# atoptima/DynamicSparseArrays.jl

Measured on AMD Instinct MI355X. Metric: spmv_gbps_10M_nnz_pcsr, higher is better.
Workload: dtype f64; 1 GPU; C3: PCSR 1000000x1000000 Float64, 10000000 nnz per GPU, dense-x SpMV y=A*x (gather over the rowmajor twin); capacity_slots=16777216, physical_slot_bytes=12, collective=none

## Files before the change

### dynamicsparsearrays.jl_amd/csrc/dsa_dev.h

```cpp
#pragma once
#include <hip/hip_runtime.h>
#include <stdint.h>
#include <functional>
#include <mutex>

namespace dsa {

constexpr int WAVE = 64;
constexpr int64_t SEM_KEY = 0;
constexpr int MAX_LEVELS = 48;
constexpr int TABLE_PEND_MAX = 1024;
constexpr int64_t VIEW_SMALL_SLOTS = 65536;

struct KeyArr {
    void* p;
    int32_t wide;
    int32_t pad_;
#if defined(__HIPCC__)
    struct Ref {
        void* p; int32_t wide; int64_t i;
        __device__ __forceinline__ operator int64_t() const {
            return wide ? static_cast<const int64_t*>(p)[i] : (int64_t) static_cast<const int32_t*>(p)[i];
        }
        __device__ __forceinline__ void operator=(int64_t k) const {
// ... 196 lines not shown
hipError_t launch_permute(KeyArr src_keys, const double* src_vals, const uint64_t* src_occ, int64_t src_cap,
                          KeyArr dst_keys, double* dst_vals, const uint64_t* dst_occ, int64_t dst_cap, int64_t n0,
                          const Op* ops, int64_t i0, int64_t* sems, RebalanceWork* wsrc, RebalanceWork* wdst, hipStream_t stream);
hipError_t launch_compact_range(KeyArr keys, const double* vals, const uint64_t* occ, int64_t from, int64_t to,
                                KeyArr out_keys, double* out_vals, int64_t out_cap, RebalanceWork* work, int64_t* count,
                                hipStream_t stream);
hipError_t launch_spx_accum(const SlotView& V, const int64_t* xi, const double* xv, int64_t nx, double* acc, uint64_t* bm, int64_t ny,
                            hipStream_t stream);
hipError_t launch_spx_repair(const SlotView& V, const double* xd, const double* xf, int64_t nx, const double* pattern, double* y, int64_t ny,
                             hipStream_t stream);
hipError_t launch_spx_pattern_bits(const double* pattern, int64_t ny, uint64_t* bm, hipStream_t stream);
hipError_t launch_spx_finish(uint64_t* bm, int64_t ny, uint32_t* tile_cnt, uint32_t* tile_off, unsigned int* ticket, double* src, int clear_src,
                             int64_t* out_i, double* out_v, int64_t cap, int64_t* d_count, long long* host, int64_t pin_cells,
                             unsigned long long seq, hipStream_t stream);
hipError_t launch_scatter_x(const int64_t* xi, const double* xv, int64_t nx, double* xd, double* xf, int64_t nxd, hipStream_t stream);
hipError_t launch_packed_equal(KeyArr ka, const double* va, KeyArr kb, const double* vb, int64_t n, int32_t* differ, hipStream_t stream);
hipError_t launch_merge_axpby(KeyArr ka, const double* va, int64_t na, double alpha, KeyArr kb, const double* vb, int64_t nb,
                              double beta, int64_t* mk, double* mv, uint64_t* keep, hipStream_t stream);
hipError_t launch_widen_keys(const void* src32, void* dst64, int64_t n, hipStream_t stream);
hipError_t launch_store_ctl(Ctl* d_ctl, const Ctl& ctl, hipStream_t stream);
hipError_t launch_init_fresh(uint64_t* occ0, uint64_t* occ1, int64_t occ_words, unsigned long long* status, int64_t status_words,
                             Ctl* d_ctl, const Ctl& ctl, hipStream_t stream);
hipError_t launch_clear_occ(uint64_t* occ, int64_t from, int64_t to, hipStream_t stream);

hipError_t pool_alloc(void** out, size_t bytes);
void pool_free(void* p);
void pool_trim(size_t keep_bytes);
size_t pool_idle_bytes();
hipError_t pinned_alloc(void** out, size_t bytes);
void pinned_free(void* p);
hipError_t stream_get(hipStream_t* out);
void stream_put(hipStream_t s, int device);

struct BuildScratch {
    int64_t n = 0;
    void* base = nullptr; hipStream_t stream = nullptr;
    void* base_val = nullptr;
    void* d_ctl = nullptr; void* h_ctl = nullptr;
    uint32_t* ghist = nullptr; uint32_t* hist = nullptr; uint32_t* cnt_c = nullptr; uint32_t* cnt_p = nullptr;
    uint64_t* comp[2] = {nullptr, nullptr}; double* val[2] = {nullptr, nullptr};
    void* queue = nullptr;
    int64_t kmin = 0, pmin = 0; int kbits = 0, pbits = 0, sorted = 0; const double* vsorted = nullptr;
    int ibits = 0;
    bool wide_path = false;
    uint32_t *idx2 = nullptr, *fpart = nullptr, *fcell = nullptr, *spart = nullptr, *scell = nullptr;
    int64_t *p2 = nullptr, *k2 = nullptr;
};
struct KeyRange { int64_t lo = 0, hi = -1; bool known() const { return hi >= lo; } };
hipError_t device_key_scan(const int64_t* d_a, const int64_t* d_b, int64_t n, KeyRange* ra, KeyRange* rb, bool* a_zero, bool* b_zero,
                           hipStream_t stream);
hipError_t launch_key_scan_acc(const int64_t* d_a, const int64_t* d_b, int64_t n, long long* d_acc, hipStream_t stream);
hipError_t build_prepare(const int64_t* d_part, const int64_t* d_key, const double* d_val, int64_t nnz, KeyRange part_range, KeyRange key_range,
                         BuildScratch& s, int64_t counts[2], hipStream_t stream, const std::function<void()>* while_sorting = nullptr);
hipError_t build_emit(const double* d_val, int32_t combine, BuildScratch& s, KeyArr out_keys, double* out_vals,
                      int64_t* part_keys, int mode, int64_t nparts_explicit, hipStream_t stream, bool wait_and_free = true,
                      uint64_t* der_comp = nullptr, double* der_val = nullptr);
hipError_t build_derived_alloc(BuildScratch& s, int64_t n, int kbits, int pbits, int64_t kmin, int64_t pmin, hipStream_t stream);
hipError_t build_derived_sort(BuildScratch& s, int64_t counts[2], hipStream_t stream, const std::function<void()>* while_sorting = nullptr);
void build_abort(BuildScratch& s);
hipError_t launch_build_small_vec(int64_t* io, int n, int cap, int32_t combine, KeyArr out_k, double* out_v, unsigned long long seq, hipStream_t stream);

hipError_t launch_sequencer(KeyArr keys, double* vals, uint64_t* occ, int64_t* sems, int64_t* col_keys,
                            uint8_t* col_live, Ctl* ctl, const Op* ops, int64_t n_ops, int64_t n_avail, bool run_ok, const uint64_t* breaks,
                            Ctl* host_ctl, unsigned long long* host_seq, unsigned int seq,
                            hipStream_t stream);
hipError_t launch_op_breaks(const Op* ops, int64_t n, int mode, uint64_t* breaks, hipStream_t stream);
hipError_t launch_make_ops(const int64_t* a, const int64_t* b, const double* v, int32_t kind, int64_t n, Op* ops, hipStream_t stream);
size_t append_run_memo_bytes();
hipError_t launch_append_run(uint64_t* occ, Ctl* ctl, int64_t i0, int64_t R, const uint64_t* flags, const int64_t* d_T,
                             uint64_t* saved_memo, const int64_t* m3_out, hipStream_t stream);
hipError_t launch_append_model3(uint64_t* occ, Ctl* ctl, int64_t R, const uint64_t* flags, const int64_t* d_T, int64_t* out, hipStream_t stream);
hipError_t launch_append_model5(uint64_t* occ, Ctl* ctl, int64_t R, const uint64_t* flags, const int64_t* d_T, int64_t* out, hipStream_t stream);
hipError_t launch_run_expand(const Op* ops, int64_t i0, int64_t R, const Ctl* ctl, int64_t* col_keys, uint8_t* col_live, Op* cells,
                             uint64_t* flags, int64_t* out, hipStream_t stream);

struct TableMerge {
    int64_t* sems2; int64_t* keys2;
    int64_t* pkey; int64_t* pdst; int64_t* psem;
    int64_t* hdr;
};
hipError_t launch_table_merge(int64_t* sems, int64_t* col_keys, uint8_t* col_live, double* vals, Ctl* ctl, TableMerge tm, int64_t table_cap,
                              hipStream_t stream);

struct Plan {
    int64_t lo, hi;
    int64_t pos, aux;
    int64_t ws, we;
    int32_t count;
    int32_t action;
};
struct RoundState {
    int64_t cursor;
    int64_t limit;
    int32_t G;
    int32_t d;
    int32_t stop;
    int32_t min_prefix, G_next, pad;
    uint32_t ticket;
    int32_t ema;
    int64_t rounds, par_ops;
    int64_t why[8];
    int32_t tight;
    int32_t seq;
    int64_t cursor_n;
    int64_t pend0;
    int32_t np, np_n;
    int32_t cur, cur_n;
    int32_t run_ahead;
    int32_t drain;
    int64_t deferred;
};
struct PendOp { int64_t op; int32_t zlo, zhi; };
struct BurstPublish { RoundState* host_rs; Ctl* host_ctl; unsigned long long* host_seq; };
constexpr int FP_MODE_SETS = 0x100, FP_MODE_SHADOW = 0x200;
constexpr size_t FP_BYTES_PER_OP = 160;
constexpr int ROUND_GMAX = 1024;
struct BurstGraph {
    hipGraphExec_t exec = nullptr; hipGraph_t graph = nullptr; hipStream_t stream = nullptr;
    const void* key[12] = {};
    bool disabled = false;
    hipStream_t failed_on = nullptr;
};
struct DevBufs { void* keys; double* vals; uint64_t* occ; int64_t* sems; int64_t* col_keys; uint8_t* col_live; int32_t wide, pad; PendOp* pend;  };
hipError_t launch_burst(const DevBufs* bufs, Ctl* ctl, const Op* ops, RoundState* rs, Plan* plans, int rounds, BurstGraph* cache,
                        BurstPublish pub, hipStream_t stream);
void burst_graph_destroy(BurstGraph* cache);
hipError_t launch_local_rounds(const DevBufs* bufs, Ctl* ctl, const Op* ops, RoundState* rs, int max_rounds, BurstPublish pub, hipStream_t stream);

hipError_t launch_get_batch(int mode, const SlotView& V, const int64_t* qa, const int64_t* qb, int64_t n, double* out, int32_t* err_out,
                            hipStream_t stream);
hipError_t launch_get_small(int mode, const SlotView& V, int64_t* io, int n, unsigned long long seq, hipStream_t stream);
enum DbgRawOp : int32_t { DBG_FIND = 0, DBG_FIND_FAST = 1, DBG_INSERT = 2, DBG_INSERT_FAST = 3, DBG_DELETE = 4, DBG_DELETE_FAST = 5,
                          DBG_PURGE = 6, DBG_REBALANCE = 7 };
hipError_t launch_dbg_raw_block(KeyArr keys, double* vals, uint64_t* occ, int64_t* sems, int64_t len, int op, int64_t key, double val,
                                int64_t from, int64_t to, int64_t m, int64_t* out, hipStream_t stream);
hipError_t launch_dbg_raw_wave(KeyArr keys, double* vals, uint64_t* occ, int64_t* sems, int64_t len, int op, int64_t key, double val,
                               int64_t from, int64_t to, int64_t m, int64_t* out, hipStream_t stream);
hipError_t launch_check(const SlotView& V, int64_t occ_words, unsigned long long* report, hipStream_t stream);
hipError_t launch_view_small(const SlotView& V, int64_t col, KeyArr out_k, double* out_v, int64_t out_cap, int64_t* meta, int64_t* host,
                             int64_t host_cells, unsigned long long seq, int64_t range_from, int64_t range_to, hipStream_t stream);
hipError_t launch_partition_range(const SlotView& V, int64_t col, int64_t* out, hipStream_t stream);

hipError_t launch_spmv_gather(const SlotView& V, const double* x, int64_t nx, double* y, int64_t ny, int pattern, int mode, hipStream_t stream);
constexpr int SPMV_ZFILL = 1;
constexpr int SPMV_PLAIN_STREAM = 2;
constexpr int64_t SPMV_SPAN_SLOTS = 512;
constexpr int SPMV_META_BLOCKS = 1024;
constexpr int SPMV_META_WORDS = 3 * SPMV_META_BLOCKS + 1;
hipError_t launch_spmv_meta(const SlotView& V, unsigned long long* scratch, unsigned long long* out6_pinned, unsigned long long seq, hipStream_t stream);
constexpr int PLAN_GROUP_SHIFT = 12;
constexpr int64_t PLAN_GROUP_SLOTS = int64_t(1) << PLAN_GROUP_SHIFT;
constexpr int PLAN_ROWS = 1024;
constexpr int PLAN_MAX_SLICES = 63;
constexpr int64_t PLAN_MAX_GROUPS = 4096;
constexpr int PLAN_DESC = 5;
struct PlanDev {
    uint32_t* cell; double* val;
    uint32_t* off;
    uint32_t* cnt;
    uint32_t* gbase;
    uint32_t* pfirst;
    uint32_t* nsem;
    uint32_t* yrow;
    int64_t groups, width, cap_cells;
    int32_t slices, pad_;
};
hipError_t launch_spmv_plan_build(const SlotView& V, int64_t nx, int64_t ny, const PlanDev& pl, unsigned long long* out3_pinned,
                                  unsigned long long seq, hipStream_t stream);
hipError_t launch_spmv_plan(const PlanDev& pl, int64_t table_len, const double* x, double* y, int64_t ny, hipStream_t stream);
hipError_t launch_spmv_scatter(const SlotView& V, const double* x, int64_t nx, double* y, int64_t ny, hipStream_t stream);

}
```

### dynamicsparsearrays.jl_amd/csrc/dsa_host.hip

```cpp
#include "host.h"

#include <dlfcn.h>

#include <algorithm>
#include <chrono>
#include <cstdlib>
#include <cstring>
#include <string>
#include <vector>

using namespace dsa;
using namespace dsa::host;

namespace {
thread_local std::string g_err;
}

namespace dsa {
namespace host {
Roctx::Roctx() {
    const char* e = getenv("DSA_ROCTX");
    if (!(e && e[0] == '1')) return;
    for (const char* n : {"librocprofiler-sdk-roctx.so.1", "librocprofiler-sdk-roctx.so", "libroctx64.so.4", "libroctx64.so"}) {
        void* lib = dlopen(n, RTLD_NOW | RTLD_GLOBAL);
        if (!lib) continue;
        push = reinterpret_cast<int (*)(const char*)>(dlsym(lib, "roctxRangePushA"));
        pop = reinterpret_cast<int (*)()>(dlsym(lib, "roctxRangePop"));
        if (push && pop) return;
        push = nullptr; pop = nullptr;
    }
}
const Roctx& roctx() { static const Roctx r; return r; }
}
}

namespace dsa {
static const char* const k_dev_switches[] = {
    "DSA_BUILD_WIDE",
    "DSA_COUNT_MODEL",
    "DSA_DBG_RUN", "DSA_DBG_SPLIT", "DSA_DBG_TIME",
    "DSA_DBG_MOVE2",
    "DSA_FAIL_BUILD",
    "DSA_FP_MODE",
    "DSA_KEYS_WIDE",
    "DSA_LOCAL_ROUNDS",
    "DSA_MODEL3",
    "DSA_MODEL5",
    "DSA_PARBATCH",
    "DSA_POS_WIDE",
    "DSA_RUN_AHEAD",
    "DSA_SPMV_PLAN",
    "DSA_SPMV_SHARE", "DSA_SPMV_STREAM",
    "DSA_SPX_XDRIVEN",
    "DSA_TIGHT",
};
const char* dev_env(const char* name) {
#ifndef NDEBUG
    bool known = false;
    for (const char* s : k_dev_switches) known = known || std::strcmp(s, name) == 0;
    if (!known) { fprintf(stderr, "dev_env: %s is not in the table of development switches\n", name); abort(); }
#endif
#ifndef DSA_DEV
    const char* on = getenv("DSA_DEV");
    if (!(on && on[0] == '1')) return nullptr;
#endif
    return getenv(name);
}

hipError_t wait_pinned_seq(const volatile void* word, uint64_t want, hipStream_t s, uint64_t mask) {
    const volatile unsigned long long* w = static_cast<const volatile unsigned long long*>(word);
    auto published = [&] { return (__atomic_load_n(w, __ATOMIC_ACQUIRE) & mask) == want; };
    auto next_query = std::chrono::steady_clock::now() + std::chrono::milliseconds(2);
    while (!published()) {
        if (std::chrono::steady_clock::now() < next_query) continue;
        const hipError_t q = hipStreamQuery(s);
        if (q == hipErrorNotReady) { next_query = std::chrono::steady_clock::now() + std::chrono::milliseconds(2); continue; }
        if (q != hipSuccess) return q;
        if (!published()) return hipErrorUnknown;
    }
    return hipSuccess;
}
void set_last_error(const char* msg) { g_err = msg ? msg : ""; }
}

namespace {

constexpr size_t PENDING_FLUSH = 1u << 16;

Pma& orient(dsa_mat* h, int32_t o) {
    if (!h->has_major) fail(DSA_EMODE, "matrix is in fill mode");
    if (o != DSA_COLMAJOR && o != DSA_ROWMAJOR) fail(DSA_EARG, "orientation must be 0 or 1");
    return o == DSA_COLMAJOR ? h->col : h->row;
}

void vec_apply(dsa_vec_t* h, const int64_t* keys, const double* vals, int64_t n) {
    int32_t err = 0;
    static const bool par = [] { const char* e = dev_env("DSA_PARBATCH"); return !(e && e[0] == '0'); }();
    int64_t done;
    if (par && n >= 128) done = run_ops_parallel(h->P, OpBatch(OP_VEC_SET, keys, nullptr, vals, n), &err);
    else {
        std::vector<Op> ops((size_t)n);
        for (int64_t i = 0; i < n; ++i) ops[(size_t)i] = make_op(OP_VEC_SET, keys[i], 0, vals[i]);
        done = run_ops(h->P, ops, &err);
    }
    const int64_t upto = err ? std::min(done + 1, n) : done;
    for (int64_t i = 0; i < upto; ++i) if (vals[i] != 0.0) h->n = std::max(h->n, keys[i]);
    if (err) fail(err, err_text(err));
}
void vec_flush(dsa_vec_t* h) {
    bind_device(h->P);
    if (h->pk.empty()) return;
    std::vector<int64_t> k; std::vector<double> v;
    k.swap(h->pk); v.swap(h->pv);
    vec_apply(h, k.data(), v.data(), (int64_t)k.size());
}

int64_t vec_pack_alt(dsa_vec_t* h) {
    Pma& P = h->P;
    int64_t cnt = 0;
    const int alt = 1 - P.cur;
    {
        const int64_t c = pack_small(P, P.K(), P.V(), P.O(), 1, P.capacity(), P.KA(alt), P.vals[alt], P.cap_alloc);
        if (c >= 0) return c;
    }
    LAUNCH("compact", launch_compact_range(P.K(), P.V(), P.O(), 1, P.capacity(), P.KA(alt), P.vals[alt], P.cap_alloc, &P.work, &cnt, P.stream));
    return cnt;
}
void wait_for_pack(dsa_vec_t* producer, dsa_vec_t* consumer) {
    if (producer->P.stream == consumer->P.stream) return;
    HIPCHK(hipStreamSynchronize(producer->P.stream));
}

dsa_vec* vec_from_packed_dev(Pma& S, int64_t n, int64_t len) {
    auto* v = new dsa_vec();
    hipStream_t own = nullptr;
    try {
        pma_init_common(v->P, false, false);
        Pma& P = v->P;
        own = P.stream; P.stream = S.stream;
        P.wide = S.wide;
        const int64_t capacity = capacity_for(n);
        set_geometry_for_new(P, capacity, n);
        ensure_capacity_alloc(P, 2 * capacity, false);
        ++P.layout_epoch; ++P.stat_grid_rebalances;
        P.h_ctl->stat_rebalances = 0; P.h_ctl->stat_window_slots = 0;
        if (capacity != P.h_ctl->segment_capacity) { P.h_ctl->stat_rebalances = 1; P.h_ctl->stat_window_slots = capacity; }
        LAUNCH("init", launch_init_fresh(P.occ[0], P.occ[1], P.occ_words, P.work.status, P.work.status_cap, P.d_ctl, *P.h_ctl, P.stream));
        const int salt = 1 - S.cur;
        LAUNCH("rebalance", launch_rebalance(S.KA(salt), S.vals[salt], S.occ[salt], 1, n, true, P.K(), P.V(), P.O(), 1, capacity, n,
                                             nullptr, &P.work, P.stream));
        P.occ_dirty[P.cur] = (capacity + 63) / 64;
        if (S.ev_handoff == nullptr) HIPCHK(hipEventCreateWithFlags(&S.ev_handoff, hipEventDisableTiming));
        HIPCHK(hipEventRecord(S.ev_handoff, S.stream));
        HIPCHK(hipStreamWaitEvent(own, S.ev_handoff, 0));
        P.stream = own;
    } catch (...) {
        if (own) { (void)hipStreamSynchronize(v->P.stream); v->P.stream = own; }
        pma_destroy(v->P); delete v; throw;
    }
    v->n = len;
    return v;
}

}

namespace dsa {
namespace host {

void ensure_xy(dsa_mat* h, int64_t nx, int64_t ny) {
    if (nx > h->x_cap) { if (h->d_x) hipFree(h->d_x); h->x_cap = std::max<int64_t>(nx, 1024); HIPCHK(hipMalloc(&h->d_x, (size_t)h->x_cap * sizeof(double))); }
    if (ny > h->y_cap) { if (h->d_y) hipFree(h->d_y); h->y_cap = std::max<int64_t>(ny, 1024); HIPCHK(hipMalloc(&h->d_y, (size_t)h->y_cap * sizeof(double))); }
}

void spmv_dev(dsa_mat* h, int32_t transpose, int32_t algo, const double* d_x, int64_t nx, double* d_y, int64_t ny, hipStream_t s,
              int pattern) {
    if (!h->has_major) fail(DSA_EMODE, "matrix is in fill mode");
    hipError_t e;
    if (algo == 0) {
        Pma& P = transpose ? h->col : h->row;
        int mode = 0;
        constexpr int64_t MAX_FILL = 4096;
        const Pma::SpmvMeta& M = spmv_meta(P);
        if (M.ordered && M.max_extent <= SPMV_SPAN_SLOTS && M.max_gap <= MAX_FILL && M.first_key >= 1 && M.first_key <= MAX_FILL &&
            ny - M.last_key <= MAX_FILL)
            { mode |= SPMV_ZFILL; ++P.stat_spmv_nomemset; }
        if (nx * (int64_t)sizeof(double) <= (3 << 20)) mode |= SPMV_PLAIN_STREAM;
        const bool plan = spmv_plan_on() && pattern == 0 && (mode & SPMV_ZFILL) && !(mode & SPMV_PLAIN_STREAM) && s == P.stream &&
                          nx > 0 && spmv_plan_shape_ok(P, nx, ny);
        if (plan && spmv_plan_product(P, d_x, nx, d_y, ny, s)) return;
        e = launch_spmv_gather(P.view(), d_x, nx, d_y, ny, pattern, mode, s);
        if (e == hipSuccess && plan && P.plan.state == Pma::SpmvPlan::NONE && P.plan.products == 2) spmv_plan_build(P, nx, ny, s);
    } else if (algo == 1) {
        Pma& P = transpose ? h->row : h->col;
        e = launch_spmv_scatter(P.view(), d_x, nx, d_y, ny, s);
    } else {
        fail(DSA_EARG, "algo must be 0 (gather) or 1 (scatter)");
    }
    launch_check(e, "spmv launch: ");
}

}
}

namespace {
// ... 732 lines not shown
```

### dynamicsparsearrays.jl_amd/csrc/spmv.hip

```cpp
#include "wave_dev.h"
#include <type_traits>

namespace dsa {

constexpr int SP_TILE = 2048;
constexpr int SP_BLOCK = 256;
constexpr int SP_WAVES = SP_BLOCK / 64;
constexpr int SP_PER_WAVE = SP_TILE / SP_WAVES;
constexpr int SP_WORDS_PER_WAVE = SP_PER_WAVE / 64;
constexpr int SP_BACK_WORDS = 32;

__device__ int64_t carry_in_partition(KeyArr keys, const double* __restrict__ vals,
                                      const uint64_t* __restrict__ occ, const int64_t* __restrict__ sems,
                                      int64_t table_len, int64_t b0) {
    const int lane = lane_id();
    int64_t w = (b0 >> 6) - 1;
    for (int it = 0; it < SP_BACK_WORDS && w >= 0; ++it, --w) {
        const uint64_t word = occ[w];
        bool issem = false;
        if ((word >> lane) & 1ull) issem = (keys[(w << 6) + lane] == SEM_KEY);
        const uint64_t b = __ballot(issem);
        if (b) {
            const int hi = 63 - __clzll(b);
            return (int64_t)vals[(w << 6) + hi];
// ... 390 lines not shown
#pragma unroll
        for (int u = 0; u < U; ++u) {
            const int64_t i = c + u * 256 + threadIdx.x;
            if (i >= table_len) continue;
            const bool last = i + 1 >= table_len;
            const int64_t e1 = last ? capacity + 1 : s1[u];
            if (s0[u] <= 0 || e1 <= s0[u]) bad = 1;
            else { const unsigned long long e = (unsigned long long)(e1 - s0[u]); ext = e > ext ? e : ext; }
            if (!last) {
                if (k1[u] <= k0[u]) bad = 1;
                else { const unsigned long long g = (unsigned long long)(k1[u] - k0[u]); gap = g > gap ? g : gap; }
            }
        }
    }
#pragma unroll
    for (int o = 32; o > 0; o >>= 1) {
        const unsigned long long e2 = __shfl_xor(ext, o, 64), g2 = __shfl_xor(gap, o, 64), b2 = __shfl_xor(bad, o, 64);
        ext = e2 > ext ? e2 : ext; gap = g2 > gap ? g2 : gap; bad |= b2;
    }
    const int lane = threadIdx.x & 63, wv = threadIdx.x >> 6;
    if (lane == 0) { sE[wv] = ext; sG[wv] = gap; sB[wv] = bad; }
    const int64_t key_first = threadIdx.x == 0 ? part_keys[0] : 0, key_last = threadIdx.x == 0 ? part_keys[table_len - 1] : 0;
    __syncthreads();
    unsigned long long* ticket = scratch + 3 * SPMV_META_BLOCKS;
    if (threadIdx.x == 0) {
        for (int w = 1; w < 4; ++w) { ext = sE[w] > ext ? sE[w] : ext; gap = sG[w] > gap ? sG[w] : gap; bad |= sB[w]; }
        __hip_atomic_store(scratch + 3 * blockIdx.x + 0, ext, __ATOMIC_RELAXED, __HIP_MEMORY_SCOPE_AGENT);
        __hip_atomic_store(scratch + 3 * blockIdx.x + 1, gap, __ATOMIC_RELAXED, __HIP_MEMORY_SCOPE_AGENT);
        __hip_atomic_store(scratch + 3 * blockIdx.x + 2, bad, __ATOMIC_RELAXED, __HIP_MEMORY_SCOPE_AGENT);
        __builtin_amdgcn_s_waitcnt(0);
        const unsigned long long t = __hip_atomic_fetch_add(ticket, 1ull, __ATOMIC_RELAXED, __HIP_MEMORY_SCOPE_AGENT);
        sLast = (t == (unsigned long long)gridDim.x - 1) ? 1u : 0u;
    }
    __syncthreads();
    if (!sLast) return;
    ext = 0; gap = 0; bad = 0;
    {
        constexpr int R = SPMV_META_BLOCKS / 256;
        unsigned long long pe[R], pg[R], pb[R];
#pragma unroll
        for (int r = 0; r < R; ++r) {
            const int b = threadIdx.x + r * 256;
            const int bc = b < (int)gridDim.x ? b : 0;
            pe[r] = __hip_atomic_load(scratch + 3 * bc + 0, __ATOMIC_RELAXED, __HIP_MEMORY_SCOPE_AGENT);
            pg[r] = __hip_atomic_load(scratch + 3 * bc + 1, __ATOMIC_RELAXED, __HIP_MEMORY_SCOPE_AGENT);
            pb[r] = __hip_atomic_load(scratch + 3 * bc + 2, __ATOMIC_RELAXED, __HIP_MEMORY_SCOPE_AGENT);
        }
#pragma unroll
        for (int r = 0; r < R; ++r) { ext = pe[r] > ext ? pe[r] : ext; gap = pg[r] > gap ? pg[r] : gap; bad |= pb[r]; }
    }
#pragma unroll
    for (int o = 32; o > 0; o >>= 1) {
        const unsigned long long e2 = __shfl_xor(ext, o, 64), g2 = __shfl_xor(gap, o, 64), b2 = __shfl_xor(bad, o, 64);
        ext = e2 > ext ? e2 : ext; gap = g2 > gap ? g2 : gap; bad |= b2;
    }
    __syncthreads();
    if (lane == 0) { sE[wv] = ext; sG[wv] = gap; sB[wv] = bad; }
    __syncthreads();
    if (threadIdx.x == 0) {
        for (int w = 1; w < 4; ++w) { ext = sE[w] > ext ? sE[w] : ext; gap = sG[w] > gap ? sG[w] : gap; bad |= sB[w]; }
        const unsigned long long r[5] = {ext, gap, (unsigned long long)key_first, (unsigned long long)key_last, bad ? 1ull : 0ull};
        for (int q = 0; q < 5; ++q) __hip_atomic_store(out + q, r[q], __ATOMIC_RELAXED, __HIP_MEMORY_SCOPE_SYSTEM);
        publish_seq(out + 5, seq);
        __hip_atomic_store(ticket, 0ull, __ATOMIC_RELAXED, __HIP_MEMORY_SCOPE_AGENT);
    }
}
hipError_t launch_spmv_meta(const SlotView& V, unsigned long long* scratch, unsigned long long* out6_pinned, unsigned long long seq,
                            hipStream_t stream) {
    const int64_t table_len = V.table_len;
    if (table_len <= 0) return hipErrorInvalidValue;
    int64_t blocks = (table_len + 1023) / 1024;
    if (blocks > 256) blocks = std::max<int64_t>(256, std::min<int64_t>(SPMV_META_BLOCKS, table_len >> 12));
    hipLaunchKernelGGL(k_spmv_meta, dim3((unsigned)blocks), dim3(256), 0, stream, V.sems, V.part_keys, table_len, V.capacity, scratch, out6_pinned, seq);
    return hipGetLastError();
}

template <bool WIDE, bool NT, bool ZFILL>
static void launch_gather_t(int64_t grid, hipStream_t stream, const SlotView& V, const double* x, int64_t nx, double* y, int64_t ny,
                            int pattern) {
    static const bool share_ok = [] { const char* e = dev_env("DSA_SPMV_SHARE"); return !(e && e[0] == '0'); }();
    const bool share = NT && share_ok && V.capacity >= SP_TILE && V.capacity % SP_TILE == 0;
    if (share)
        hipLaunchKernelGGL((k_spmv_gather<WIDE, NT, ZFILL, true>), dim3((unsigned)grid), dim3(SP_BLOCK), 0, stream, V.keys, V.vals, V.occ,
                           V.capacity, V.sems, V.part_keys, V.table_len, x, nx, y, ny, pattern);
    else
        hipLaunchKernelGGL((k_spmv_gather<WIDE, NT, ZFILL, false>), dim3((unsigned)grid), dim3(SP_BLOCK), 0, stream, V.keys, V.vals, V.occ,
                           V.capacity, V.sems, V.part_keys, V.table_len, x, nx, y, ny, pattern);
}

static hipError_t launch_spmv(bool scatter, int pattern, int mode, const SlotView& V, const double* x, int64_t nx, double* y, int64_t ny,
                              hipStream_t stream) {
    {
        static const char* st = dev_env("DSA_SPMV_STREAM"); if (st) mode = (mode & ~2) | (st[0] == 'p' ? 2 : 0);
    }
    if (scatter) mode = 0;
    const bool zfill = (mode & 1) && V.table_len > 0;
    if (!zfill) {
        hipError_t e = hipMemsetAsync(y, 0, (size_t)ny * sizeof(double), stream);
        if (e != hipSuccess) return e;
    }
    const int64_t ntiles = (V.capacity + SP_TILE - 1) / SP_TILE;
    const int64_t grid = ntiles >= 64 ? 8 * ((ntiles + 7) / 8) : ntiles;
    if (scatter) {
        hipLaunchKernelGGL(k_spmv_scatter, dim3((unsigned)grid), dim3(SP_BLOCK), 0, stream, V.keys, V.vals, V.occ, V.capacity, V.sems,
                           V.part_keys, V.table_len, x, nx, y, ny, 0);
        return hipGetLastError();
    }
    const int sel = (V.keys.wide ? 4 : 0) | ((mode & 2) ? 0 : 2) | (zfill ? 1 : 0);
#define DSA_GATHER_CASE(W_, N_, Z_) launch_gather_t<W_, N_, Z_>(grid, stream, V, x, nx, y, ny, pattern)
    switch (sel) {
        case 0: DSA_GATHER_CASE(false, false, false); break;
        case 1: DSA_GATHER_CASE(false, false, true); break;
        case 2: DSA_GATHER_CASE(false, true, false); break;
        case 3: DSA_GATHER_CASE(false, true, true); break;
        case 4: DSA_GATHER_CASE(true, false, false); break;
        case 5: DSA_GATHER_CASE(true, false, true); break;
        case 6: DSA_GATHER_CASE(true, true, false); break;
        default: DSA_GATHER_CASE(true, true, true); break;
    }
#undef DSA_GATHER_CASE
    return hipGetLastError();
}

constexpr uint32_t PLAN_NONE = 0xffffffffu;

template <bool SCATTER>
__global__ __launch_bounds__(256) void k_plan_pass(KeyArr keys, const double* __restrict__ vals, const uint64_t* __restrict__ occ,
                                                   int64_t capacity, int64_t nx, PlanDev pl,
                                                   const int64_t* __restrict__ part_keys, int64_t table_len, int64_t ny) {
    __shared__ uint32_t sPos[SP_WAVES][PLAN_MAX_SLICES + 1];
    const int lane = threadIdx.x & 63, wv = threadIdx.x >> 6;
    const int64_t g = (int64_t)blockIdx.x * SP_WAVES + wv;
    if (g >= pl.groups) return;
    uint32_t* pos = sPos[wv];
    const int P = pl.slices;
    const uint32_t W = (uint32_t)pl.width;
    if (SCATTER) {
        const uint32_t c = lane < P ? pl.cnt[g * P + lane] : 0u;
        uint32_t incl = c;
#pragma unroll
        for (int o = 1; o < 64; o <<= 1) { const uint32_t t = __shfl_up(incl, o, 64); if (lane >= o) incl += t; }
        const uint32_t start = pl.gbase[g] + incl - c;
        uint32_t* __restrict__ drow = pl.off + g * (P + PLAN_DESC);
        const uint32_t p0 = pl.pfirst[g], np = pl.pfirst[g + 1] - p0;
        if (lane <= P) { pos[lane] = start; drow[PLAN_DESC - 1 + lane] = start; }
        const int64_t top = ny + 1;
        auto clamped = [&](int64_t k) -> uint32_t { return (uint32_t)(k < 0 ? 0 : (k > top ? top : k)); };
        bool dense = true;
        for (uint32_t i = (uint32_t)lane; i < np; i += 64u) {
            const int64_t id = (int64_t)p0 + i;
            if (id < table_len) {
                const uint32_t k = clamped(part_keys[id]), kp = id > 0 ? clamped(part_keys[id - 1]) : 0u;
                pl.yrow[id] = k;
                dense = dense && k == kp + 1u && k >= 1u && (int64_t)k <= ny && (id + 1 < table_len || (int64_t)k == ny);
            } else dense = false;
        }
        const bool all_dense = __ballot(!dense) == 0ull && np > 0u;
        if (lane == 0) {
            drow[0] = p0; drow[1] = np;
            drow[2] = (int64_t)p0 < table_len ? clamped(part_keys[p0]) : 0u;
            drow[3] = all_dense ? 1u : 0u;
        }
    } else {
        pos[lane] = 0u;
    }
    __builtin_amdgcn_wave_barrier();
    const int64_t nwords = (capacity + 63) >> 6;
    const int64_t wg0 = g << (PLAN_GROUP_SHIFT - 6);
    const int64_t wg1 = wg0 + (PLAN_GROUP_SLOTS >> 6) < nwords ? wg0 + (PLAN_GROUP_SLOTS >> 6) : nwords;
    const uint64_t le = mask_lt(lane) | (1ull << lane);
    int nsem = 0;
    for (int64_t w = wg0; w < nwords; ++w) {
        const bool tail = w >= wg1;
        if (tail && nsem == 0) break;
        const uint64_t word = occ[w];
        const bool bit = (word >> lane) & 1ull;
        int64_t key = -1;
        double v = 0.0;
        if (bit) { key = keys[(w << 6) + lane]; if (SCATTER) v = vals[(w << 6) + lane]; }
        const uint64_t sm = __ballot(bit && key == SEM_KEY);
        int row;
        bool cell;
        if (!tail) {
            row = nsem + popc64(sm & le) - 1;
            cell = bit && key != SEM_KEY && row >= 0;
            nsem += popc64(sm);
        } else {
            const int lim = sm ? __ffsll((unsigned long long)sm) - 1 : 64;
            row = nsem - 1;
            cell = bit && lane < lim;
        }
        cell = cell && key >= 1 && key <= nx;
        const uint32_t col0 = cell ? (uint32_t)(key - 1) : 0u;
        const uint32_t s = col0 / W;
        uint64_t todo = __ballot(cell);
        while (todo) {
            const int leader = __ffsll((unsigned long long)todo) - 1;
            const uint32_t s0 = (uint32_t)__builtin_amdgcn_readlane((int)s, leader);
            const bool mine = cell && s == s0;
            const uint64_t m = __ballot(mine);
            const uint32_t base = pos[s0];
            if (SCATTER && mine) {
                const uint32_t idx = base + (uint32_t)popc64(m & mask_lt(lane));
                if ((int64_t)idx < pl.cap_cells) {
                    __builtin_nontemporal_store(((uint32_t)row << 16) | (col0 - s0 * W), pl.cell + idx);
                    __builtin_nontemporal_store(v, pl.val + idx);
                }
            }
            __builtin_amdgcn_wave_barrier();
            if (lane == 0) pos[s0] = base + (uint32_t)popc64(m);
            __builtin_amdgcn_wave_barrier();
            todo &= ~m;
        }
        if (tail && sm) break;
    }
    if (!SCATTER) {
        if (lane < P) pl.cnt[g * P + lane] = pos[lane];
        if (lane == 0) pl.nsem[g] = (uint32_t)nsem;
    }
}

constexpr int PLAN_SCAN_THREADS = 1024;
__global__ __launch_bounds__(PLAN_SCAN_THREADS) void k_plan_scan(PlanDev pl, int64_t table_len, unsigned long long* __restrict__ out,
                                                                 unsigned long long seq) {
    constexpr int PER = PLAN_MAX_GROUPS / PLAN_SCAN_THREADS;
    __shared__ unsigned long long sTot[PLAN_SCAN_THREADS], sSem[PLAN_SCAN_THREADS];
    __shared__ unsigned int sBad;
    const int t = threadIdx.x;
    const int P = pl.slices;
    if (t == 0) sBad = 0u;
    unsigned long long tot[PER], sem[PER], ts = 0, ss = 0;
    bool bad = false;
#pragma unroll
    for (int q = 0; q < PER; ++q) {
        const int64_t g = (int64_t)t * PER + q;
        tot[q] = 0; sem[q] = 0;
        if (g < pl.groups) {
            for (int s = 0; s < P; ++s) tot[q] += pl.cnt[g * P + s];
            sem[q] = pl.nsem[g];
            bad = bad || sem[q] > (unsigned long long)PLAN_ROWS;
        }
        ts += tot[q]; ss += sem[q];
    }
    sTot[t] = ts; sSem[t] = ss;
    __syncthreads();
    if (bad) atomicOr(&sBad, 1u);
    for (int o = 1; o < PLAN_SCAN_THREADS; o <<= 1) {
        const unsigned long long a = t >= o ? sTot[t - o] : 0ull, b = t >= o ? sSem[t - o] : 0ull;
        __syncthreads();
        sTot[t] += a; sSem[t] += b;
        __syncthreads();
    }
    unsigned long long rt = sTot[t] - ts, rs = sSem[t] - ss;
#pragma unroll
    for (int q = 0; q < PER; ++q) {
        const int64_t g = (int64_t)t * PER + q;
        if (g < pl.groups) { pl.gbase[g] = (uint32_t)rt; pl.pfirst[g] = (uint32_t)rs; }
        rt += tot[q]; rs += sem[q];
    }
    if (t == PLAN_SCAN_THREADS - 1) {
        const unsigned long long cells = sTot[t], parts = sSem[t];
        pl.pfirst[pl.groups] = (uint32_t)parts;
        const bool ok = sBad == 0u && (long long)cells <= pl.cap_cells && (long long)parts == table_len && cells < 0xffffffffull;
        __hip_atomic_store(out + 0, ok ? 1ull : 0ull, __ATOMIC_RELAXED, __HIP_MEMORY_SCOPE_SYSTEM);
        __hip_atomic_store(out + 1, cells, __ATOMIC_RELAXED, __HIP_MEMORY_SCOPE_SYSTEM);
        publish_seq(out + 2, seq);
    }
}

hipError_t launch_spmv_plan_build(const SlotView& V, int64_t nx, int64_t ny, const PlanDev& pl, unsigned long long* out3_pinned,
                                  unsigned long long seq, hipStream_t stream) {
    if (pl.groups <= 0 || pl.groups > PLAN_MAX_GROUPS || pl.slices <= 0 || pl.slices > PLAN_MAX_SLICES || pl.width <= 0 || pl.width > 65536 ||
        ny < 0 || ny + 1 >= ((int64_t)1 << 32))
        return hipErrorInvalidValue;
    const unsigned grid = (unsigned)((pl.groups + SP_WAVES - 1) / SP_WAVES);
    hipLaunchKernelGGL(k_plan_pass<false>, dim3(grid), dim3(SP_BLOCK), 0, stream, V.keys, V.vals, V.occ, V.capacity, nx, pl, V.part_keys,
                       V.table_len, ny);
    hipLaunchKernelGGL(k_plan_scan, dim3(1), dim3(PLAN_SCAN_THREADS), 0, stream, pl, V.table_len, out3_pinned, seq);
    hipLaunchKernelGGL(k_plan_pass<true>, dim3(grid), dim3(SP_BLOCK), 0, stream, V.keys, V.vals, V.occ, V.capacity, nx, pl, V.part_keys,
                       V.table_len, ny);
    return hipGetLastError();
}

constexpr int PLAN_U = 1;
__global__ __launch_bounds__(SP_BLOCK) void k_spmv_plan(PlanDev pl, int64_t table_len, const double* __restrict__ x,
                                                        double* __restrict__ y, int64_t ny) {
    __shared__ double sAcc[SP_WAVES][PLAN_ROWS];
    const int lane = threadIdx.x & 63, wv = threadIdx.x >> 6;
    const int64_t g = (int64_t)blockIdx.x * SP_WAVES + wv;
    if (g >= pl.groups) return;
    double* acc = sAcc[wv];
    const int P = pl.slices;
    const uint32_t W = (uint32_t)pl.width;
    const uint32_t* __restrict__ cp = pl.cell;
    const double* __restrict__ vp = pl.val;
    const uint32_t* __restrict__ drow = pl.off + g * (P + PLAN_DESC);
    const uint32_t dH = drow[lane & 3];
    const uint32_t myoff = drow[PLAN_DESC - 1 + (lane < P ? lane : P)];
#pragma unroll
    for (int k = 0; k < PLAN_ROWS / 64; ++k) acc[k * 64 + lane] = 0.0;
    const uint32_t p0 = (uint32_t)__builtin_amdgcn_readlane((int)dH, 0);
    const int np = __builtin_amdgcn_readlane((int)dH, 1);
    const uint32_t row0 = (uint32_t)__builtin_amdgcn_readlane((int)dH, 2);
    const bool dense = __builtin_amdgcn_readlane((int)dH, 3) != 0;
    auto off_at = [&](int j) -> uint32_t { return (uint32_t)__builtin_amdgcn_readlane((int)myoff, j); };
    __builtin_amdgcn_wave_barrier();

    auto load_round = [&](uint32_t b, uint32_t e, uint32_t (&c)[PLAN_U], double (&v)[PLAN_U]) {
#pragma unroll
        for (int u = 0; u < PLAN_U; ++u) {
            const uint32_t i = b + u * 64 + lane;
            c[u] = PLAN_NONE; v[u] = 0.0;
            if (i < e) { c[u] = cp[i]; v[u] = vp[i]; }
        }
    };
    auto gather = [&](uint32_t base, const uint32_t (&c)[PLAN_U], double (&xq)[PLAN_U]) {
#pragma unroll
        for (int u = 0; u < PLAN_U; ++u) xq[u] = x[c[u] != PLAN_NONE ? base + (c[u] & 0xffffu) : 0u];
    };
    auto apply = [&](const uint32_t (&c)[PLAN_U], const double (&v)[PLAN_U], const double (&xq)[PLAN_U]) {
#pragma unroll
        for (int u = 0; u < PLAN_U; ++u) {
            const bool valid = c[u] != PLAN_NONE;
            if (__ballot(valid) == 0ull) break;
            const uint32_t row = c[u] >> 16;
            const double p = v[u] * xq[u];
            const uint32_t prow = (uint32_t)__shfl_up((int)row, 1, 64);
            const uint64_t heads = __ballot(valid && (lane == 0 || prow != row));
            const int rank = lane - (63 - __clzll(heads & (mask_lt(lane) | (1ull << lane))));
            for (int r = 0;; ++r) {
                if (valid && rank == r && row < (uint32_t)PLAN_ROWS) acc[row] = acc[row] + p;
                __builtin_amdgcn_wave_barrier();
                if (__ballot(valid && rank > r) == 0ull) break;
            }
        }
    };

    uint32_t cA[PLAN_U], cB[PLAN_U];
    double vA[PLAN_U], vB[PLAN_U], xq[PLAN_U];
#pragma unroll
    for (int u = 0; u < PLAN_U; ++u) { cB[u] = PLAN_NONE; vB[u] = 0.0; }
    uint32_t b = off_at(0), e = off_at(1);
    load_round(b, e, cA, vA);
    uint32_t r = b;
    for (int s = 0;;) {
        gather((uint32_t)s * W, cA, xq);
        uint32_t nr = r + PLAN_U * 64;
        int ns = s;
        if (nr >= e) {
            ns = s + 1;
            if (ns < P) { nr = off_at(ns); e = off_at(ns + 1); }
        }
        const bool more = ns < P;
        if (more) load_round(nr, e, cB, vB);
        apply(cA, vA, xq);
        if (!more) break;
#pragma unroll
        for (int u = 0; u < PLAN_U; ++u) { cA[u] = cB[u]; vA[u] = vB[u]; }
        r = nr; s = ns;
    }
    __builtin_amdgcn_wave_barrier();
    if (dense) {
        for (int i = lane; i < np; i += 64) y[row0 - 1u + (uint32_t)i] = acc[i];
        return;
    }
    const uint32_t ny32 = (uint32_t)ny, last_id = (uint32_t)table_len - 1u;
    for (int i = lane; i < np; i += 64) {
        const uint32_t id = p0 + (uint32_t)i;
        const uint32_t row = pl.yrow[id], prev = id > 0u ? pl.yrow[id - 1u] : 0u;
        if (prev < row) for (uint32_t q = prev + 1u; q < row; ++q) y[q - 1u] = 0.0;
        if (id == last_id && row < ny32) for (uint32_t q = row + 1u; q <= ny32; ++q) y[q - 1u] = 0.0;
        if (row >= 1u && row <= ny32) y[row - 1u] = acc[i];
    }
}

hipError_t launch_spmv_plan(const PlanDev& pl, int64_t table_len, const double* x, double* y, int64_t ny, hipStream_t stream) {
    if (pl.groups <= 0 || pl.groups > PLAN_MAX_GROUPS) return hipErrorInvalidValue;
    const unsigned grid = (unsigned)((pl.groups + SP_WAVES - 1) / SP_WAVES);
    hipLaunchKernelGGL(k_spmv_plan, dim3(grid), dim3(SP_BLOCK), 0, stream, pl, table_len, x, y, ny);
    return hipGetLastError();
}

hipError_t launch_spmv_gather(const SlotView& V, const double* x, int64_t nx, double* y, int64_t ny, int pattern, int mode, hipStream_t stream) {
    return launch_spmv(false, pattern, mode, V, x, nx, y, ny, stream);
}
hipError_t launch_spmv_scatter(const SlotView& V, const double* x, int64_t nx, double* y, int64_t ny, hipStream_t stream) {
    return launch_spmv(true, 0, 0, V, x, nx, y, ny, stream);
}

}
```

### dynamicsparsearrays.jl_amd/csrc/spmv_host.hip

```cpp
#include "host.h"

#include <algorithm>
#include <chrono>
#include <cstring>

namespace dsa {
namespace host {

static bool spmv_meta_applicable(const Pma& P) {
    const Ctl& c = *P.h_ctl;
    return P.has_cols && c.table_len > 0 && P.view().dense && c.n_pending == 0;
}
void prefetch_spmv_meta(Pma& P) {
    if (P.spmv_meta.epoch == P.layout_epoch || P.meta_inflight_epoch == P.layout_epoch || !spmv_meta_applicable(P)) return;
    if (!P.d_meta) {
        HIPCHK(hipMalloc(&P.d_meta, SPMV_META_WORDS * sizeof(unsigned long long)));
        HIPCHK(hipMemsetAsync(P.d_meta, 0, SPMV_META_WORDS * sizeof(unsigned long long), P.stream));
        HIPCHK(pinned_alloc(reinterpret_cast<void**>(&P.h_meta), 16 * sizeof(int64_t)));
        std::memset(P.h_meta, 0, 16 * sizeof(int64_t));
        P.meta_seq = 0;
    }
    LAUNCH("spmv meta", launch_spmv_meta(P.view(), P.d_meta,
                                         reinterpret_cast<unsigned long long*>(P.h_meta), ++P.meta_seq, P.stream));
    P.meta_inflight_epoch = P.layout_epoch;
}
const Pma::SpmvMeta& spmv_meta(Pma& P) {
    Pma::SpmvMeta& M = P.spmv_meta;
    if (M.epoch == P.layout_epoch) return M;
    M = Pma::SpmvMeta();
    M.epoch = P.layout_epoch;
    if (!spmv_meta_applicable(P)) return M;
    M.epoch = -1;
    prefetch_spmv_meta(P);
    wait_policy_block(P);
    volatile int64_t* seqp = P.h_meta + 5;
    const auto t0 = std::chrono::steady_clock::now();
    bool synced = false;
    while ((unsigned long long)__atomic_load_n(seqp, __ATOMIC_ACQUIRE) != P.meta_seq) {
        if (!synced && std::chrono::steady_clock::now() - t0 > std::chrono::milliseconds(1)) { HIPCHK(hipStreamSynchronize(P.stream)); synced = true; continue; }
        if (synced) fail(DSA_EHIP, "SpMV meta kernel finished without publishing its result");
    }
    M.epoch = P.layout_epoch;
    const int64_t* r = P.h_meta;
    M.ordered = r[4] == 0;
    M.max_extent = r[0]; M.max_gap = r[1]; M.first_key = r[2]; M.last_key = r[3];
    return M;
}

bool spmv_plan_on() { static const bool on = [] { const char* e = dev_env("DSA_SPMV_PLAN"); return !(e && e[0] == '0'); }(); return on; }

void spmv_plan_drop(Pma& P) {
    Pma::SpmvPlan& L = P.plan;
    if (L.mem[0] || L.mem[1]) {
        if (P.stream) (void)hipStreamSynchronize(P.stream);
        pool_free(L.mem[0]); pool_free(L.mem[1]);
    }
    const unsigned long long seq = L.seq;
    L = Pma::SpmvPlan();
    L.seq = seq;
}

static int plan_slices(int64_t nx) { return (int)std::max<int64_t>(16, (nx + 65535) / 65536); }

bool spmv_plan_shape_ok(const Pma& P, int64_t nx, int64_t ny) {
    const int64_t groups = (P.capacity() + PLAN_GROUP_SLOTS - 1) / PLAN_GROUP_SLOTS;
    return groups <= PLAN_MAX_GROUPS && plan_slices(nx) <= PLAN_MAX_SLICES && P.h_ctl->nb_elements < ((int64_t)1 << 31) &&
           ny >= 0 && ny + 1 < ((int64_t)1 << 32);
}

void spmv_plan_build(Pma& P, int64_t nx, int64_t ny, hipStream_t s) {
    Pma::SpmvPlan& L = P.plan;
    PlanDev& d = L.dev;
    d.groups = (P.capacity() + PLAN_GROUP_SLOTS - 1) / PLAN_GROUP_SLOTS;
    d.slices = plan_slices(nx);
    d.width = (nx + d.slices - 1) / d.slices;
    d.cap_cells = std::max<int64_t>(1, P.h_ctl->nb_elements - P.h_ctl->table_len);
    const int64_t G = d.groups, S = d.slices;
    const int64_t T = std::max<int64_t>(1, P.h_ctl->table_len);
    const int64_t words = G * (S + PLAN_DESC) + G * S + G + (G + 1) + G + T;
    HIPCHK(pool_alloc(&L.mem[0], (size_t)d.cap_cells * (sizeof(uint32_t) + sizeof(double))));
    HIPCHK(pool_alloc(&L.mem[1], (size_t)words * sizeof(uint32_t)));
    L.bytes = d.cap_cells * 12 + words * 4;
    d.val = static_cast<double*>(L.mem[0]);
    d.cell = reinterpret_cast<uint32_t*>(d.val + d.cap_cells);
    d.off = static_cast<uint32_t*>(L.mem[1]);
    d.cnt = d.off + G * (S + PLAN_DESC);
    d.gbase = d.cnt + G * S;
    d.pfirst = d.gbase + G;
    d.nsem = d.pfirst + G + 1;
    d.yrow = d.nsem + G;
    unsigned long long* out = reinterpret_cast<unsigned long long*>(P.h_meta + 6);
    launch_check(launch_spmv_plan_build(P.view(), nx, ny, d, out, ++L.seq, s), "spmv plan build: ");
    L.state = Pma::SpmvPlan::PENDING;
    ++P.stat_spmv_plan_builds;
}

bool spmv_plan_product(Pma& P, const double* d_x, int64_t nx, double* d_y, int64_t ny, hipStream_t s) {
    Pma::SpmvPlan& L = P.plan;
    if (L.content_epoch != P.content_epoch || L.layout_epoch != P.layout_epoch || L.nx != nx || L.ny != ny) {
        spmv_plan_drop(P);
        L.content_epoch = P.content_epoch; L.layout_epoch = P.layout_epoch; L.nx = nx; L.ny = ny;
    }
    ++L.products;
    if (L.state == Pma::SpmvPlan::PENDING) {
        HIPCHK(wait_pinned_seq(P.h_meta + 8, L.seq, s));
        const bool ok = __atomic_load_n(P.h_meta + 6, __ATOMIC_ACQUIRE) == 1;
        if (ok) L.state = Pma::SpmvPlan::USABLE;
        else {
            const int64_t ce = L.content_epoch, le = L.layout_epoch, pr = L.products;
            spmv_plan_drop(P);
            L.content_epoch = ce; L.layout_epoch = le; L.nx = nx; L.ny = ny; L.products = pr;
            L.state = Pma::SpmvPlan::UNUSABLE;
        }
    }
    if (L.state == Pma::SpmvPlan::USABLE) {
        LAUNCH("spmv plan", launch_spmv_plan(L.dev, P.h_ctl->table_len, d_x, d_y, ny, s));
        ++P.stat_spmv_plan;
        return true;
    }
    return false;
}

}
}
```

Measured before the change: 4970 GB/s.

## Write sparse-row outputs via a row-presence bitmap and split plan SpMV into passes

The plan build now records which output rows are present in a bitmap, and the plan SpMV's non-dense store path walks that bitmap word by word with wave-wide readlanes. Each lane then writes either the accumulated value or a zero, replacing per-row serial zero-fill loops that could stall a single lane on long gaps. The plan SpMV launch is also split into passes of at most 4096 groups, which lets plans with up to 16384 groups use the fast path instead of falling back. The cost is an extra bitmap plus a memset and atomics during build, and extra kernel launches when the group count is large.

```diff
diff --git a/dynamicsparsearrays.jl_amd/csrc/dsa_dev.h b/dynamicsparsearrays.jl_amd/csrc/dsa_dev.h
--- a/dynamicsparsearrays.jl_amd/csrc/dsa_dev.h
+++ b/dynamicsparsearrays.jl_amd/csrc/dsa_dev.h
@@ -372,7 +372,14 @@
 constexpr int64_t PLAN_GROUP_SLOTS = int64_t(1) << PLAN_GROUP_SHIFT;
 constexpr int PLAN_ROWS = 1024;
 constexpr int PLAN_MAX_SLICES = 63;
-constexpr int64_t PLAN_MAX_GROUPS = 4096;
+constexpr int64_t PLAN_LAUNCH_GROUPS = 4096;
+constexpr int64_t PLAN_MAX_GROUPS = 16384;
+constexpr int PLAN_PASS_ALIGN = 4;
+inline int64_t plan_pass_groups(int64_t G, int64_t per_launch) {
+    const int64_t passes = (G + per_launch - 1) / per_launch;
+    const int64_t n = passes > 0 ? (G + passes - 1) / passes : 0;
+    return (n + PLAN_PASS_ALIGN - 1) / PLAN_PASS_ALIGN * PLAN_PASS_ALIGN;
+}
 constexpr int PLAN_DESC = 5;
 struct PlanDev {
     uint32_t* cell; double* val;
@@ -382,6 +389,7 @@
     uint32_t* pfirst;
     uint32_t* nsem;
     uint32_t* yrow;
+    uint64_t* ybits;
     int64_t groups, width, cap_cells;
     int32_t slices, pad_;
 };
diff --git a/dynamicsparsearrays.jl_amd/csrc/dsa_host.hip b/dynamicsparsearrays.jl_amd/csrc/dsa_host.hip
--- a/dynamicsparsearrays.jl_amd/csrc/dsa_host.hip
+++ b/dynamicsparsearrays.jl_amd/csrc/dsa_host.hip
@@ -50,6 +50,7 @@
     "DSA_POS_WIDE",
     "DSA_RUN_AHEAD",
     "DSA_SPMV_PLAN",
+    "DSA_SPMV_PLAN_PASS",
     "DSA_SPMV_SHARE", "DSA_SPMV_STREAM",
     "DSA_SPX_XDRIVEN",
     "DSA_TIGHT",
diff --git a/dynamicsparsearrays.jl_amd/csrc/spmv.hip b/dynamicsparsearrays.jl_amd/csrc/spmv.hip
--- a/dynamicsparsearrays.jl_amd/csrc/spmv.hip
+++ b/dynamicsparsearrays.jl_amd/csrc/spmv.hip
@@ -566,6 +566,7 @@
             if (id < table_len) {
                 const uint32_t k = clamped(part_keys[id]), kp = id > 0 ? clamped(part_keys[id - 1]) : 0u;
                 pl.yrow[id] = k;
+                if (k >= 1u && (int64_t)k <= ny) atomicOr(reinterpret_cast<unsigned long long*>(pl.ybits) + ((k - 1u) >> 6), 1ull << ((k - 1u) & 63u));
                 dense = dense && k == kp + 1u && k >= 1u && (int64_t)k <= ny && (id + 1 < table_len || (int64_t)k == ny);
             } else dense = false;
         }
@@ -635,9 +636,9 @@
 }
 
 constexpr int PLAN_SCAN_THREADS = 1024;
+template <int PER>
 __global__ __launch_bounds__(PLAN_SCAN_THREADS) void k_plan_scan(PlanDev pl, int64_t table_len, unsigned long long* __restrict__ out,
                                                                  unsigned long long seq) {
-    constexpr int PER = PLAN_MAX_GROUPS / PLAN_SCAN_THREADS;
     __shared__ unsigned long long sTot[PLAN_SCAN_THREADS], sSem[PLAN_SCAN_THREADS];
     __shared__ unsigned int sBad;
     const int t = threadIdx.x;
@@ -690,7 +691,13 @@
     const unsigned grid = (unsigned)((pl.groups + SP_WAVES - 1) / SP_WAVES);
     hipLaunchKernelGGL(k_plan_pass<false>, dim3(grid), dim3(SP_BLOCK), 0, stream, V.keys, V.vals, V.occ, V.capacity, nx, pl, V.part_keys,
                        V.table_len, ny);
-    hipLaunchKernelGGL(k_plan_scan, dim3(1), dim3(PLAN_SCAN_THREADS), 0, stream, pl, V.table_len, out3_pinned, seq);
+    static_assert(PLAN_LAUNCH_GROUPS % PLAN_SCAN_THREADS == 0 && PLAN_MAX_GROUPS % PLAN_SCAN_THREADS == 0, "groups per scan thread");
+    if (pl.groups <= PLAN_LAUNCH_GROUPS)
+        hipLaunchKernelGGL(k_plan_scan<PLAN_LAUNCH_GROUPS / PLAN_SCAN_THREADS>, dim3(1), dim3(PLAN_SCAN_THREADS), 0, stream, pl, V.table_len,
+                           out3_pinned, seq);
+    else
+        hipLaunchKernelGGL(k_plan_scan<PLAN_MAX_GROUPS / PLAN_SCAN_THREADS>, dim3(1), dim3(PLAN_SCAN_THREADS), 0, stream, pl, V.table_len,
+                           out3_pinned, seq);
     hipLaunchKernelGGL(k_plan_pass<true>, dim3(grid), dim3(SP_BLOCK), 0, stream, V.keys, V.vals, V.occ, V.capacity, nx, pl, V.part_keys,
                        V.table_len, ny);
     return hipGetLastError();
@@ -698,11 +705,11 @@
 
 constexpr int PLAN_U = 1;
 __global__ __launch_bounds__(SP_BLOCK) void k_spmv_plan(PlanDev pl, int64_t table_len, const double* __restrict__ x,
-                                                        double* __restrict__ y, int64_t ny) {
+                                                        double* __restrict__ y, int64_t ny, int64_t g_first, int64_t g_end) {
     __shared__ double sAcc[SP_WAVES][PLAN_ROWS];
     const int lane = threadIdx.x & 63, wv = threadIdx.x >> 6;
-    const int64_t g = (int64_t)blockIdx.x * SP_WAVES + wv;
-    if (g >= pl.groups) return;
+    const int64_t g = g_first + (int64_t)blockIdx.x * SP_WAVES + wv;
+    if (g >= g_end) return;
     double* acc = sAcc[wv];
     const int P = pl.slices;
     const uint32_t W = (uint32_t)pl.width;
@@ -778,20 +785,47 @@
         for (int i = lane; i < np; i += 64) y[row0 - 1u + (uint32_t)i] = acc[i];
         return;
     }
-    const uint32_t ny32 = (uint32_t)ny, last_id = (uint32_t)table_len - 1u;
-    for (int i = lane; i < np; i += 64) {
-        const uint32_t id = p0 + (uint32_t)i;
-        const uint32_t row = pl.yrow[id], prev = id > 0u ? pl.yrow[id - 1u] : 0u;
-        if (prev < row) for (uint32_t q = prev + 1u; q < row; ++q) y[q - 1u] = 0.0;
-        if (id == last_id && row < ny32) for (uint32_t q = row + 1u; q <= ny32; ++q) y[q - 1u] = 0.0;
-        if (row >= 1u && row <= ny32) y[row - 1u] = acc[i];
+    if (np <= 0) return;
+    const uint32_t ny32 = (uint32_t)ny, idl = p0 + (uint32_t)np - 1u;
+    const uint32_t kprev = p0 > 0u ? pl.yrow[p0 - 1u] : 0u, klast = pl.yrow[idl];
+    const uint32_t lo = kprev;
+    const uint32_t hi = (idl == (uint32_t)table_len - 1u || klast > ny32) ? ny32 : klast;
+    if (hi <= lo) return;
+    const uint32_t w0 = lo >> 6, w1 = (hi - 1u) >> 6;
+    int base = 0;
+    for (uint32_t wb = w0; wb <= w1; wb += 64u) {
+        const uint32_t wi = wb + (uint32_t)lane;
+        unsigned long long mine = wi <= w1 ? pl.ybits[wi] : 0ull;
+        if (wi == w0) mine &= ~mask_lt((int)(lo & 63u));
+        const int n = w1 - wb + 1u < 64u ? (int)(w1 - wb + 1u) : 64;
+        for (int k = 0; k < n; ++k) {
+            const unsigned long long word = ((unsigned long long)(uint32_t)__builtin_amdgcn_readlane((int)(mine >> 32), k) << 32) |
+                                            (uint32_t)__builtin_amdgcn_readlane((int)(uint32_t)mine, k);
+            const uint32_t r = ((wb + (uint32_t)k) << 6) + (uint32_t)lane;
+            const int idx = base + popc64(word & mask_lt(lane));
+            const bool has = ((word >> lane) & 1ull) != 0ull && idx < np;
+            if (r >= lo && r < hi) y[r] = has ? acc[idx] : 0.0;
+            base += popc64(word);
+        }
     }
 }
 
 hipError_t launch_spmv_plan(const PlanDev& pl, int64_t table_len, const double* x, double* y, int64_t ny, hipStream_t stream) {
+    static_assert(PLAN_PASS_ALIGN == SP_WAVES && PLAN_LAUNCH_GROUPS % PLAN_PASS_ALIGN == 0, "a pass is a whole number of workgroups");
     if (pl.groups <= 0 || pl.groups > PLAN_MAX_GROUPS) return hipErrorInvalidValue;
-    const unsigned grid = (unsigned)((pl.groups + SP_WAVES - 1) / SP_WAVES);
-    hipLaunchKernelGGL(k_spmv_plan, dim3(grid), dim3(SP_BLOCK), 0, stream, pl, table_len, x, y, ny);
+    static const int64_t per_launch = [] {
+        const char* e = dev_env("DSA_SPMV_PLAN_PASS");
+        if (!e) return PLAN_LAUNCH_GROUPS;
+        const long long v = atoll(e);
+        return v >= PLAN_PASS_ALIGN && v <= PLAN_LAUNCH_GROUPS && v % PLAN_PASS_ALIGN == 0 ? (int64_t)v : (int64_t)-1;
+    }();
+    if (per_launch < 0) return hipErrorInvalidValue;
+    const int64_t n = plan_pass_groups(pl.groups, per_launch);
+    for (int64_t g0 = 0; g0 < pl.groups; g0 += n) {
+        const int64_t g1 = g0 + n < pl.groups ? g0 + n : pl.groups;
+        hipLaunchKernelGGL(k_spmv_plan, dim3((unsigned)((g1 - g0 + SP_WAVES - 1) / SP_WAVES)), dim3(SP_BLOCK), 0, stream, pl, table_len, x, y,
+                           ny, g0, g1);
+    }
     return hipGetLastError();
 }
 
diff --git a/dynamicsparsearrays.jl_amd/csrc/spmv_host.hip b/dynamicsparsearrays.jl_amd/csrc/spmv_host.hip
--- a/dynamicsparsearrays.jl_amd/csrc/spmv_host.hip
+++ b/dynamicsparsearrays.jl_amd/csrc/spmv_host.hip
@@ -77,13 +77,16 @@
     d.cap_cells = std::max<int64_t>(1, P.h_ctl->nb_elements - P.h_ctl->table_len);
     const int64_t G = d.groups, S = d.slices;
     const int64_t T = std::max<int64_t>(1, P.h_ctl->table_len);
-    const int64_t words = G * (S + PLAN_DESC) + G * S + G + (G + 1) + G + T;
+    const int64_t B = std::max<int64_t>(1, (ny + 63) / 64);
+    const int64_t words = 2 * B + G * (S + PLAN_DESC) + G * S + G + (G + 1) + G + T;
     HIPCHK(pool_alloc(&L.mem[0], (size_t)d.cap_cells * (sizeof(uint32_t) + sizeof(double))));
     HIPCHK(pool_alloc(&L.mem[1], (size_t)words * sizeof(uint32_t)));
     L.bytes = d.cap_cells * 12 + words * 4;
+    d.ybits = static_cast<uint64_t*>(L.mem[1]);
+    HIPCHK(hipMemsetAsync(d.ybits, 0, (size_t)B * sizeof(uint64_t), s));
     d.val = static_cast<double*>(L.mem[0]);
     d.cell = reinterpret_cast<uint32_t*>(d.val + d.cap_cells);
-    d.off = static_cast<uint32_t*>(L.mem[1]);
+    d.off = static_cast<uint32_t*>(L.mem[1]) + 2 * B;
     d.cnt = d.off + G * (S + PLAN_DESC);
     d.gbase = d.cnt + G * S;
     d.pfirst = d.gbase + G;
```

Result: no change. 4969 GB/s (-0.0%).
